# nelaturuharsha/TurboPrune

Hardware: NVIDIA H100
Metric: images_per_sec_resnet50_erk80_train_step (higher is better)
Workload: dtype bf16

## Files before the change

### include/turboprune_b200.h

```cpp
#ifndef TURBOPRUNE_B200_H
#define TURBOPRUNE_B200_H

#include <stddef.h>
#include <stdint.h>

#ifdef __cplusplus
extern "C" {
#endif

#define TP_OK                 0
#define TP_ERR_INVALID       -1
#define TP_ERR_WORKSPACE     -2
#define TP_ERR_CUDA          -3
#define TP_ERR_K_RANGE       -4
#define TP_ERR_UNSUPPORTED   -5
#define TP_ERR_DEVICE        -6

const char* tp_strerror(int code);
const char* tp_last_cuda_error(void);
int         tp_abi_version(void);
int         tp_device_sm_count(void);
int         tp_set_pdl(int on);

#define TP_SCORE_MAG      0
// ... 51 lines not shown
int tp_synth_normal(void* out, int64_t numel, uint64_t seed, uint64_t counter_offset, int raw_words, void* stream);
int tp_synth_labels(void* out, int64_t numel, int num_classes, uint64_t seed, uint64_t counter_offset, void* stream);

typedef struct tp_conv_desc {
  int32_t n, h, w, cin;
  int32_t cout, r, s;
  int32_t stride_h, stride_w, pad_h, pad_w;
  int32_t p, q;
} tp_conv_desc;

size_t tp_conv_workspace_bytes(const tp_conv_desc* d, int op);

int tp_conv_fprop(const tp_conv_desc* d, const void* x, const void* wf, const void* bias_f32,
                  void* y, void* ws, size_t ws_bytes, void* stream);
size_t tp_conv_stats_rows(const tp_conv_desc* d);
int tp_conv_fprop_stats(const tp_conv_desc* d, const void* x, const void* wf, const void* kmask_f, const void* bias_f32,
                        void* y, void* stats, void* ws, size_t ws_bytes, void* stream);
int tp_conv_dgrad(const tp_conv_desc* d, const void* dy, const void* wd, const void* kmask_d, const void* addend,
                  void* dx, void* ws, size_t ws_bytes, void* stream);
size_t tp_conv_dgrad_partial_rows(const tp_conv_desc* d);
int tp_conv_dgrad_bnrelu(const tp_conv_desc* d, const void* dy, const void* wd, const void* kmask_d,
                         const void* bn_y, const void* bn_weight, const void* bn_bias, const void* bn_mean, const void* bn_invstd,
                         void* g, void* partial, void* stream);
int tp_conv_wgrad(const tp_conv_desc* d, const void* x, const void* dy, const void* mask, const void* kmask_f,
                  int cin_real, void* dw, void* db, void* ws, size_t ws_bytes, void* stream);

int tp_bn_forward_ext(const void* y, const void* residual, void* z, int64_t M, int C,
                      const void* weight, const void* bias, void* running_mean, void* running_var,
                      void* num_batches_tracked, float momentum, float eps, int training, int relu,
                      void* save_mean, void* save_invstd, const void* ext_stats, int64_t ext_rows,
                      void* ws, size_t ws_bytes, void* stream);

size_t tp_bn_workspace_bytes(int64_t m, int c);
int tp_bn_forward(const void* y, const void* residual, void* z, int64_t m, int c,
                  const void* weight, const void* bias, void* running_mean, void* running_var,
                  void* num_batches_tracked, float momentum, float eps, int training, int relu,
                  void* save_mean, void* save_invstd, void* ws, size_t ws_bytes, void* stream);
int tp_bn_backward(const void* dz, const void* z, const void* y, int64_t m, int c, const void* weight, const void* bias,
                   const void* save_mean, const void* save_invstd, int relu, void* dy, void* dres,
                   void* dweight, void* dbias, void* ws, size_t ws_bytes, void* stream);

int tp_bn_backward_ext(const void* g, const void* y, int64_t M, int C, const void* weight, const void* bias,
                       const void* save_mean, const void* save_invstd, const void* partial_rows, int64_t n_rows,
                       void* dy, void* dweight, void* dbias, void* ws, size_t ws_bytes, void* stream);
int tp_maxpool_forward(const void* x, void* y, void* idx, int n, int h, int w, int c, int k, int stride, int pad,
                       int p, int q, void* stream);
// ... 21 lines not shown
```

### turboprune_b200/_cabi.py

```python
import ctypes
import os
from ctypes import POINTER, c_char_p, c_float, c_int, c_int32, c_int64, c_size_t, c_uint64, c_void_p

from . import build as _build

TP_SCORE_MAG, TP_SCORE_SNIP, TP_SCORE_SYNFLOW = 0, 1, 2
TP_ERR_K_RANGE = -4

_lib = None


class ConvDesc(ctypes.Structure):
    _fields_ = [(n, c_int32) for n in
                ("n", "h", "w", "cin", "cout", "r", "s", "stride_h", "stride_w", "pad_h", "pad_w", "p", "q")]


class StageItem(ctypes.Structure):
    _fields_ = [("w", c_void_p), ("mask", c_void_p), ("wf", c_void_p), ("wd", c_void_p)] + \
               [(n, c_int32) for n in ("cout", "cin", "r", "s", "cin_p", "cout_p", "wf_ld")] + \
               [("kmask_f", c_void_p), ("kmask_d", c_void_p)]


SIGNATURES = {
    "tp_strerror": (c_char_p, [c_int]),
# ... 12 lines not shown
    "tp_apply_threshold": (c_int, [POINTER(c_void_p), POINTER(c_void_p), POINTER(c_void_p), POINTER(c_void_p),
                                   POINTER(c_int64), c_int, c_int, c_void_p, c_void_p, c_size_t, c_void_p]),
    "tp_count_zeros": (c_int, [POINTER(c_void_p), POINTER(c_int64), c_int, c_void_p, c_void_p, c_size_t, c_void_p]),
    "tp_stage_weights": (c_int, [c_void_p, c_void_p, c_int, c_int, c_int, c_int, c_void_p, c_int, c_int, c_void_p, c_int,
                                 c_int, c_void_p, c_void_p, c_void_p]),
    "tp_kblock_mask_words": (c_size_t, [c_int64]),
    "tp_stage_batched_workspace_bytes": (c_size_t, [c_int]),
    "tp_stage_weights_batched": (c_int, [POINTER(StageItem), c_int, c_int, c_void_p, c_size_t, c_void_p, c_size_t, c_void_p]),
    "tp_to_nhwc_bf16": (c_int, [c_void_p, c_int, c_int64, c_int64, c_int64, c_int64, c_int, c_int, c_int, c_int,
                                c_void_p, c_int, c_void_p]),
    "tp_im2col_c8": (c_int, [c_void_p] + [c_int] * 11 + [c_void_p, c_int, c_void_p]),
    "tp_im2col_stem": (c_int, [c_void_p, c_int, c_int64, c_int64, c_int64, c_int64] + [c_int] * 13 + [c_void_p, c_int, c_void_p]),
    "tp_cifar_augment": (c_int, [c_void_p, c_void_p, c_void_p, c_void_p, c_void_p, c_void_p, c_int, c_int, c_int, c_int, c_int, c_int, c_void_p]),
    "tp_synth_normal": (c_int, [c_void_p, c_int64, c_uint64, c_uint64, c_int, c_void_p]),
    "tp_synth_labels": (c_int, [c_void_p, c_int64, c_int, c_uint64, c_uint64, c_void_p]),
    "tp_conv_workspace_bytes": (c_size_t, [POINTER(ConvDesc), c_int]),
    "tp_conv_fprop": (c_int, [POINTER(ConvDesc), c_void_p, c_void_p, c_void_p, c_void_p, c_void_p, c_size_t, c_void_p]),
    "tp_conv_stats_rows": (c_size_t, [POINTER(ConvDesc)]),
    "tp_conv_fprop_stats": (c_int, [POINTER(ConvDesc), c_void_p, c_void_p, c_void_p, c_void_p, c_void_p, c_void_p, c_void_p, c_size_t, c_void_p]),
    "tp_conv_dgrad": (c_int, [POINTER(ConvDesc), c_void_p, c_void_p, c_void_p, c_void_p, c_void_p, c_void_p, c_size_t, c_void_p]),
    "tp_conv_dgrad_partial_rows": (c_size_t, [POINTER(ConvDesc)]),
    "tp_conv_dgrad_bnrelu": (c_int, [POINTER(ConvDesc), c_void_p, c_void_p, c_void_p, c_void_p, c_void_p, c_void_p, c_void_p, c_void_p,
                                     c_void_p, c_void_p, c_void_p]),
    "tp_bn_backward_ext": (c_int, [c_void_p, c_void_p, c_int64, c_int, c_void_p, c_void_p, c_void_p, c_void_p, c_void_p, c_int64,
                                   c_void_p, c_void_p, c_void_p, c_void_p, c_size_t, c_void_p]),
    "tp_conv_wgrad": (c_int, [POINTER(ConvDesc), c_void_p, c_void_p, c_void_p, c_void_p, c_int, c_void_p, c_void_p, c_void_p,
                              c_size_t, c_void_p]),
    "tp_sgd_momentum": (c_int, [POINTER(c_void_p), POINTER(c_void_p), POINTER(c_void_p), POINTER(c_int64), c_int,
                                c_void_p, c_float, c_float, c_int, c_int, c_void_p, c_size_t, c_void_p]),
    "tp_segtable_workspace_bytes": (c_size_t, [c_int]),
    "tp_p2p_allreduce_mask": (c_int, [POINTER(c_void_p), POINTER(c_void_p), c_int, c_int, c_int64, c_void_p, c_float,
                                      c_void_p, c_int, c_int, c_void_p, c_void_p]),
    "tp_bn_workspace_bytes": (c_size_t, [c_int64, c_int]),
    "tp_bn_forward": (c_int, [c_void_p, c_void_p, c_void_p, c_int64, c_int, c_void_p, c_void_p, c_void_p, c_void_p, c_void_p,
                              c_float, c_float, c_int, c_int, c_void_p, c_void_p, c_void_p, c_size_t, c_void_p]),
    "tp_bn_forward_ext": (c_int, [c_void_p, c_void_p, c_void_p, c_int64, c_int, c_void_p, c_void_p, c_void_p, c_void_p, c_void_p,
                                  c_float, c_float, c_int, c_int, c_void_p, c_void_p, c_void_p, c_int64, c_void_p, c_size_t, c_void_p]),
    "tp_bn_backward": (c_int, [c_void_p, c_void_p, c_void_p, c_int64, c_int, c_void_p, c_void_p, c_void_p, c_void_p, c_int, c_void_p,
                               c_void_p, c_void_p, c_void_p, c_void_p, c_size_t, c_void_p]),
    "tp_maxpool_forward": (c_int, [c_void_p, c_void_p, c_void_p] + [c_int] * 9 + [c_void_p]),
    "tp_maxpool_backward": (c_int, [c_void_p, c_void_p, c_void_p] + [c_int] * 9 + [c_void_p]),
    "tp_p2p_allreduce_nvls": (c_int, [POINTER(c_void_p), POINTER(c_void_p), c_void_p, c_int, c_int, c_int64, c_void_p, c_float,
                                      c_void_p, c_int, c_void_p, c_void_p]),
}


# ... 59 lines not shown
```

### turboprune_b200/csrc/tp_core.cu

```cuda
#include "tp_common.cuh"
#include <stdlib.h>
#include <string.h>
#include <vector>

namespace tp {

static thread_local char g_last_err[512] = "";

void set_last_cuda_error(cudaError_t e, const char* where) {
  snprintf(g_last_err, sizeof(g_last_err), "%s: %s (%s)", where, cudaGetErrorName(e), cudaGetErrorString(e));
}

static int g_pdl = -1;
bool pdl_enabled() {
  if (g_pdl < 0) { const char* e = getenv("TP_PDL"); g_pdl = (e && e[0] == '1') ? 1 : 0; }
  return g_pdl == 1;
}

int sm_count() {
  static int cached[64] = {0};
  int dev = 0;
  if (cudaGetDevice(&dev) != cudaSuccess || dev < 0 || dev >= 64) return 132;
  if (cached[dev] == 0) {
    int n = 0;
// ... 52 lines not shown
  if (tiles_out) *tiles_out = tile;
  if (total_out) *total_out = start;
  return TP_OK;
}

}

extern "C" {

const char* tp_strerror(int code) {
  switch (code) {
    case TP_OK: return "ok";
    case TP_ERR_INVALID: return "invalid argument";
    case TP_ERR_WORKSPACE: return "workspace too small";
    case TP_ERR_CUDA: return "CUDA error (see tp_last_cuda_error)";
    case TP_ERR_K_RANGE: return "kthvalue(): selected number k out of range";
    case TP_ERR_UNSUPPORTED: return "unsupported configuration";
    case TP_ERR_DEVICE: return "device is not sm_90 (H100)";
    default: return "unknown error";
  }
}

const char* tp_last_cuda_error(void) { return tp::g_last_err; }
int tp_abi_version(void) { return 8; }
int tp_device_sm_count(void) { return tp::sm_count(); }
int tp_set_pdl(int on) { const int prev = tp::pdl_enabled() ? 1 : 0; tp::g_pdl = on ? 1 : 0; return prev; }

size_t tp_segtable_workspace_bytes(int n_seg) {
  return tp::align_up(sizeof(tp::Seg) * (size_t)(n_seg > 0 ? n_seg : 1), 256) + 256;
}

}
```

### turboprune_b200/csrc/tp_igemm.cu

```cuda
#include "tp_common.cuh"
#include "tp_ptx.cuh"
#include <cuda.h>
#include <mutex>

namespace tp {
using namespace ptx;

constexpr int kBlockM = 128;
constexpr int kBlockK = 64;
constexpr int kConsumers = 256;
constexpr int kThreads = kConsumers + 32;
constexpr int kProducerWarp = kConsumers / 32;
constexpr int kMaxTaps = 64;

__host__ __device__ constexpr int fwd_stages(int block_n) { return block_n == 128 ? 4 : 6; }
__host__ __device__ constexpr int fwd_tail(int block_n) { return kBlockM * block_n * 4 + 8 * 32 * 128 + 1024 + 512; }

struct TapEntry { uint16_t off_w, off_h; int32_t kofs; };

constexpr int kMaxCls = 4;

struct ClsEntry {
  int M;
  int P_it, Q_it;
// ... 3 lines not shown
  int tile0, m_groups;
};

struct FwdParams {
  int M, N;
  int ncls;
  ClsEntry cls[kMaxCls];
  int cchunks;
  int a_mode;
  int step_w, step_h;
  long long out_img_pix;
  int out_row_pix;
  int osh, osw;
  int linear;
  int ws_stages, ws_b_bytes;
  int ldc;
  int tma_store;
  __nv_bfloat16* out;
  const float* bias;
  const __nv_bfloat16* addend;
  float* stats;
  const __nv_bfloat16* bn_y;
  const float* bn_weight; const float* bn_bias; const float* bn_mean; const float* bn_invstd;
  const uint32_t* kmask;
  int kmask_words;
  TapEntry taps[kMaxTaps];
};

__device__ __forceinline__ const uint32_t* live_kmask(const uint32_t* km, int words, int N) {
#ifdef TP_NO_KMASK
  return nullptr;
#else
  if (km && __ldg(km + (size_t)((N + 63) >> 6) * words) == 0u) return nullptr;
  return km;
#endif
}

struct KSkip {
  const uint32_t* base; int words, g0, g1; int cur_w; uint32_t bits;
  __device__ __forceinline__ void begin(const uint32_t* km, int wds, int n0, int block_n, int N) {
    base = km; words = wds; cur_w = -1; bits = 0u;
    g0 = n0 >> 6; g1 = min((min(n0 + block_n, N) + 63) >> 6, ((N + 63) >> 6));
  }
  __device__ __forceinline__ bool on(int kb) {
    const int wi = kb >> 5;
    if (wi != cur_w) {
// ... 33 lines not shown
}

struct AMaps { CUtensorMap m[kMaxCls]; };

__device__ __forceinline__ void decode_tile(const FwdParams& p, int tile, int n_tiles, int& c, int& m_g, int& n_t) {
  c = 0;
#pragma unroll
  for (int j = 1; j < kMaxCls; ++j) if (j < p.ncls && tile >= p.cls[j].tile0) c = j;
  const int local = tile - p.cls[c].tile0;
  m_g = local / n_tiles; n_t = local - m_g * n_tiles;
}

template <int BLOCK_N>
__device__ __forceinline__ void fwd_mma_block(float (&acc)[BLOCK_N / 2], uint32_t a_addr, uint32_t b_addr, uint32_t accumulate) {
  const uint64_t adesc = make_smem_desc(a_addr, 16, 1024);
  const uint64_t bdesc = make_smem_desc(b_addr, 16, 1024);
#pragma unroll
  for (int k = 0; k < kBlockK / 16; ++k) {
    if constexpr (BLOCK_N == 128) wgmma_m64n128<0, 0>(acc, adesc + (uint64_t)(2 * k), bdesc + (uint64_t)(2 * k), accumulate | (uint32_t)k);
    else wgmma_m64n64<0, 0>(acc, adesc + (uint64_t)(2 * k), bdesc + (uint64_t)(2 * k), accumulate | (uint32_t)k);
  }
}

template <int BLOCK_N, bool MULTI, bool WS, bool BNB>
__global__ void __launch_bounds__(kThreads, 1)
k_igemm_fwd(const __grid_constant__ AMaps tmA, const __grid_constant__ CUtensorMap tmB,
            const __grid_constant__ FwdParams p) {
  static_assert(BLOCK_N == 64 || BLOCK_N == 128, "wgmma N of the fwd kernel");
  static_assert(!WS || !MULTI, "weight-stationary walk: single class");
  static_assert(!BNB || (!MULTI && !WS), "BatchNorm-backward epilogue: single class, default walk");
  constexpr int kABytes = kBlockM * kBlockK * 2;
  constexpr int kBBytes = BLOCK_N * kBlockK * 2;
  constexpr int kStageBytes = kABytes + kBBytes;
  constexpr int kStages = fwd_stages(BLOCK_N);
  extern __shared__ __align__(1024) uint8_t smem_raw[];
  uint8_t* smem = (uint8_t*)(((uintptr_t)smem_raw + 1023) & ~(uintptr_t)1023);
  pdl_trigger();
  constexpr int kStgBytes = 32 * 128;
  constexpr int kMaxStages = 16;
  const int n_stages = WS ? p.ws_stages : kStages;
  const int a_stride = WS ? kABytes : kStageBytes;
  uint8_t* const a_base = WS ? smem + p.ws_b_bytes : smem;
  float* const acc_tile = (float*)(a_base + n_stages * a_stride);
  uint8_t* stg_base = (uint8_t*)(acc_tile + kBlockM * BLOCK_N);
  uint64_t* full_bar = (uint64_t*)(stg_base + 8 * kStgBytes);
  uint64_t* empty_bar = full_bar + (WS ? kMaxStages : kStages);
  uint64_t* bres_bar = empty_bar + (WS ? kMaxStages : kStages);

  const int warp = threadIdx.x >> 5, lane = threadIdx.x & 31;
  const int n_tiles = (p.N + BLOCK_N - 1) / BLOCK_N;
  const int total_tiles = p.cls[p.ncls - 1].tile0 + p.cls[p.ncls - 1].m_groups * n_tiles;
  const int ws_nt = WS ? (int)blockIdx.x % n_tiles : 0;
  const int ws_m0 = WS ? (int)blockIdx.x / n_tiles : 0, ws_dm = WS ? (int)gridDim.x / n_tiles : 1;
// ... 182 lines not shown
            const int r = r0 + 8 * h, col = 8 * j + 2 * (lane & 3);
            *reinterpret_cast<float2*>(acc_tile + r * BLOCK_N + (((col >> 2) ^ (r & 7)) << 2) + (col & 3)) =
                make_float2(acc[4 * j + 2 * h], acc[4 * j + 2 * h + 1]);
          }
        bar_sync(1, kConsumers);
      }
      if (p.tma_store) {
        const uint32_t buf = smem_u32(stg_base + warp * kStgBytes);
        __nv_bfloat16* const gout = p.out;
        const __nv_bfloat16* const gadd = p.addend;
        {
        const float* bias = p.bias;
        float* stats = p.stats ? p.stats + (long long)(m_t * 4 + quarter) * 2 * N + c16 * 8 : nullptr;
        const uint32_t wr_base = buf + lane * 128;
        const uint32_t wr_sw = (uint32_t)(lane & 7);
        const uint32_t rd_even = buf + r_in * 128 + ((uint32_t)(c16 ^ r_in) << 4);
        const uint32_t rd_odd = buf + (r_in + 4) * 128 + ((uint32_t)(c16 ^ (r_in + 4)) << 4);
        uint4 a_pref[8];
#pragma unroll 1
        for (int c = half * 64; c < BLOCK_N; c += 128) {
          const int n0 = n_t * BLOCK_N + c;
          if (n0 >= N) break;
          const bool col_ok = n0 + c16 * 8 + 8 <= N;
          uint32_t v[64];
          acc_row_ld(c, v);
          acc_row_ld(c + 32, v + 32);
          if (gadd) {
            if (c == half * 64) {
#pragma unroll
              for (int i = 0; i < 8; ++i) {
                a_pref[i] = make_uint4(0u, 0u, 0u, 0u);
                if (i * 4 + r_in < rows_left && col_ok) a_pref[i] = *reinterpret_cast<const uint4*>(gadd + row_off(i) + n0);
              }
            }
#pragma unroll
            for (int i = 0; i < 8; ++i) sts128(((i & 1) ? rd_odd : rd_even) + (uint32_t)((i >> 1) * 1024), a_pref[i]);
            if (c + 128 < BLOCK_N && n0 + 128 < N) {
              const bool col_ok2 = n0 + 128 + c16 * 8 + 8 <= N;
#pragma unroll
              for (int i = 0; i < 8; ++i) {
                a_pref[i] = make_uint4(0u, 0u, 0u, 0u);
                if (i * 4 + r_in < rows_left && col_ok2) a_pref[i] = *reinterpret_cast<const uint4*>(gadd + row_off(i) + n0 + 128);
              }
            }
            __syncwarp();
          }
// ... 64 lines not shown
                  const float2 y2 = __bfloat1622float2(yh[q]);
                  if (!(fmaf(y2.x, sc[2 * q], sf[2 * q]) > 0.f)) d2.x = 0.f;
                  if (!(fmaf(y2.y, sc[2 * q + 1], sf[2 * q + 1]) > 0.f)) d2.y = 0.f;
                  gh[q] = __floats2bfloat162_rn(d2.x, d2.y);
                  s1[2 * q] += d2.x;     s2[2 * q] = fmaf(d2.x, (y2.x - nm[2 * q]) * is_[2 * q], s2[2 * q]);
                  s1[2 * q + 1] += d2.y; s2[2 * q + 1] = fmaf(d2.y, (y2.y - nm[2 * q + 1]) * is_[2 * q + 1], s2[2 * q + 1]);
                }
              }
            }
#pragma unroll
            for (int i = 0; i < 8; ++i)
              if (i * 4 + r_in < rows_left && col_ok) *reinterpret_cast<uint4*>(gout + row_off(i) + n0) = o[i];
#pragma unroll
            for (int q = 0; q < 8; ++q) {
              s1[q] += __shfl_xor_sync(0xffffffffu, s1[q], 8);  s2[q] += __shfl_xor_sync(0xffffffffu, s2[q], 8);
              s1[q] += __shfl_xor_sync(0xffffffffu, s1[q], 16); s2[q] += __shfl_xor_sync(0xffffffffu, s2[q], 16);
            }
            if (r_in == 0 && col_ok) {
              float4* d1 = reinterpret_cast<float4*>(stats + n0);
              float4* d2 = reinterpret_cast<float4*>(stats + N + n0);
              d1[0] = make_float4(s1[0], s1[1], s1[2], s1[3]); d1[1] = make_float4(s1[4], s1[5], s1[6], s1[7]);
              d2[0] = make_float4(s2[0], s2[1], s2[2], s2[3]); d2[1] = make_float4(s2[4], s2[5], s2[6], s2[7]);
            }
          } else {
#pragma unroll
          for (int i = 0; i < 8; ++i)
            if (i * 4 + r_in < rows_left && col_ok) *reinterpret_cast<uint4*>(gout + row_off(i) + n0) = o[i];
          if (stats) {
            float s1[8], s2[8];
#pragma unroll
            for (int q = 0; q < 8; ++q) { s1[q] = 0.f; s2[q] = 0.f; }
#pragma unroll
            for (int i = 0; i < 8; ++i) {
              if (i * 4 + r_in < rows_left) {
                const __nv_bfloat162* h2 = reinterpret_cast<const __nv_bfloat162*>(&o[i]);
#pragma unroll
                for (int q = 0; q < 4; ++q) {
                  const float2 t2 = __bfloat1622float2(h2[q]);
                  s1[2 * q] += t2.x; s2[2 * q] = fmaf(t2.x, t2.x, s2[2 * q]);
                  s1[2 * q + 1] += t2.y; s2[2 * q + 1] = fmaf(t2.y, t2.y, s2[2 * q + 1]);
                }
              }
            }
#pragma unroll
            for (int q = 0; q < 8; ++q) {
              s1[q] += __shfl_xor_sync(0xffffffffu, s1[q], 8);  s2[q] += __shfl_xor_sync(0xffffffffu, s2[q], 8);
// ... 377 lines not shown
static int pick_block_n(long long m_tiles, int n) {
  const int sms = sm_count();
  if (const char* e = getenv("TP_IGEMM_BN")) {
    const int f = atoi(e);
    if ((f == 64 || f == 128) && (f == 64 || n > f / 2)) return f;
  }
  int best = 64; double best_score = -1;
  const int cands[2] = {128, 64};
  const double weight[2] = {1.0, 0.82};
  for (int i = 0; i < 2; ++i) {
    int bn = cands[i];
    if (bn > 64 && n <= bn / 2) continue;
    long long tiles = m_tiles * ((n + bn - 1) / bn);
    long long waves = (tiles + sms - 1) / sms;
    double eff = (double)tiles / (double)(waves * sms) * weight[i];
    if (eff > best_score) { best_score = eff; best = bn; }
  }
  return best;
}

constexpr int kSmemMax = 232448;
constexpr int kWsMinStages = 3;

template <int BN, bool MULTI, bool WS, bool BNB = false>
static int launch_fwd(const AMaps& a, const CUtensorMap& b, FwdParams& p, cudaStream_t st) {
  constexpr int kStages = fwd_stages(BN);
  constexpr int kTail = fwd_tail(BN);
  int smem = kStages * (kBlockM * kBlockK * 2 + BN * kBlockK * 2) + kTail;
  static_assert(fwd_stages(BN) * (kBlockM * kBlockK * 2 + BN * kBlockK * 2) + fwd_tail(BN) <= kSmemMax, "fwd smem budget");
  const int n_tiles = (p.N + BN - 1) / BN;
  if (WS) {
    p.ws_b_bytes = p.cls[0].ntaps * p.cchunks * BN * kBlockK * 2;
    p.ws_stages = (kSmemMax - kTail - p.ws_b_bytes) / (kBlockM * kBlockK * 2);
    if (p.ws_stages > 16) p.ws_stages = 16;
    if (p.ws_stages < kWsMinStages) return TP_ERR_UNSUPPORTED;
    smem = p.ws_b_bytes + p.ws_stages * kBlockM * kBlockK * 2 + kTail;
  }
  static bool attr_set = false;
  if (!attr_set) {
    TP_CUDA_CHECK(cudaFuncSetAttribute(k_igemm_fwd<BN, MULTI, WS, BNB>, cudaFuncAttributeMaxDynamicSharedMemorySize, WS ? kSmemMax : smem));
    attr_set = true;
  }
  long long ctiles = 0;
  for (int c = 0; c < p.ncls; ++c) {
    p.cls[c].m_groups = (int)((p.cls[c].M + kBlockM - 1) / kBlockM);
    if (ctiles > 0x7fffffffll) return TP_ERR_UNSUPPORTED;
    p.cls[c].tile0 = (int)ctiles;
    ctiles += (long long)p.cls[c].m_groups * n_tiles;
  }
  if (ctiles > 0x7fffffffll || ctiles <= 0) return TP_ERR_UNSUPPORTED;
  int grid = (int)(ctiles < sm_count() ? ctiles : sm_count());
  if (WS) grid = (sm_count() / n_tiles) * n_tiles;
  TP_CUDA_CHECK(launch(k_igemm_fwd<BN, MULTI, WS, BNB>, dim3(grid), dim3(kThreads), (size_t)smem, st, a, b, p));
  TP_LAUNCH_CHECK();
  return TP_OK;
}

static int run_fwd(const AMaps& a, const CUtensorMap& b, FwdParams& p, int bn, cudaStream_t st) {
  p.linear = p.ncls == 1 && p.osh == 1 && p.osw == 1 && p.cls[0].oah == 0 && p.cls[0].oaw == 0 &&
             p.out_row_pix == p.cls[0].Q_it && p.out_img_pix == (long long)p.cls[0].P_it * p.cls[0].Q_it;
  p.tma_store = (p.ldc % 8 == 0 && p.N % 8 == 0 && (((uintptr_t)p.out) & 15) == 0 &&
                 (!p.addend || (((uintptr_t)p.addend) & 15) == 0)) ? 1 : 0;
  if (p.stats && !(p.tma_store && p.linear)) return TP_ERR_UNSUPPORTED;
  const bool multi = !p.linear;
  if (multi) {
    if (bn == 128) return launch_fwd<128, true, false>(a, b, p, st);
    return launch_fwd<64, true, false>(a, b, p, st);
  }
  if (p.bn_y) {
    if (!p.tma_store || !p.stats) return TP_ERR_UNSUPPORTED;
    if (bn == 128) return launch_fwd<128, false, false, true>(a, b, p, st);
    return launch_fwd<64, false, false, true>(a, b, p, st);
  }
  const int n_tiles = (p.N + bn - 1) / bn;
  const long long m_tiles = (p.cls[0].M + kBlockM - 1) / kBlockM;
  const long long b_bytes = (long long)p.cls[0].ntaps * p.cchunks * bn * kBlockK * 2;
  const long long ws_max_b = (long long)kSmemMax - (bn == 128 ? fwd_tail(128) : fwd_tail(64)) - kWsMinStages * kBlockM * kBlockK * 2;
  const char* e = getenv("TP_IGEMM_WS");
  const bool ws = e && atoi(e) != 0 && b_bytes <= ws_max_b && n_tiles <= sm_count() / 2 && m_tiles >= 4ll * (sm_count() / n_tiles);
  if (ws) {
    if (bn == 128) return launch_fwd<128, false, true>(a, b, p, st);
    return launch_fwd<64, false, true>(a, b, p, st);
  }
  if (bn == 128) return launch_fwd<128, false, false>(a, b, p, st);
  return launch_fwd<64, false, false>(a, b, p, st);
}

template <int NB>
static int launch_wgrad(int grid, const CUtensorMap& ta, const CUtensorMap& tb, const WgParams& p, cudaStream_t st) {
  constexpr int smem = 4 * (kBlockM * kBlockK * 2 + 4 * 64 * kBlockK * 2) + 1024 + 256;
// ... 67 lines not shown
    TapEntry& t = p.taps[r * d->s + s];
    t.off_w = (uint16_t)s; t.off_h = (uint16_t)r; t.kofs = (r * d->s + s) * d->cin;
  }
  AMaps ta; CUtensorMap tb;
  if (is_plain_gemm(d)) {
    p.a_mode = 0;
    rc = make_tiled_map(&ta.m[0], x, (uint64_t)d->cin, (uint64_t)p.M, (uint64_t)d->cin, kBlockM); if (rc) return rc;
  } else {
    p.a_mode = 1;
    ce.base_w = -d->pad_w; ce.base_h = -d->pad_h; p.step_w = d->stride_w; p.step_h = d->stride_h;
    rc = make_im2col_map(&ta.m[0], x, d->n, d->h, d->w, d->cin, ce.base_w, ce.base_h, p.step_w, p.step_h, d->p, d->q, kBlockM);
    if (rc) return rc;
  }
  for (int c = 1; c < kMaxCls; ++c) ta.m[c] = ta.m[0];
  const int bn = pick_block_n((p.M + kBlockM - 1) / kBlockM, p.N);
  rc = make_tiled_map(&tb, wf, (uint64_t)d->r * d->s * d->cin, (uint64_t)d->cout, (uint64_t)d->r * d->s * d->cin, (uint32_t)bn);
  if (rc) return rc;
  return run_fwd(ta, tb, p, bn, st);
}

struct BnGate { const void* y; const float* weight; const float* bias; const float* mean; const float* invstd; float* partial; };

static int conv_dgrad_impl(const tp_conv_desc* d, const void* dy, const void* wd, const void* kmask_d, const void* addend,
                           void* dx, const BnGate* gate, void* stream);

int tp_conv_dgrad(const tp_conv_desc* d, const void* dy, const void* wd, const void* kmask_d, const void* addend,
                  void* dx, void* ws, size_t ws_bytes, void* stream) {
  (void)ws; (void)ws_bytes;
  return conv_dgrad_impl(d, dy, wd, kmask_d, addend, dx, nullptr, stream);
}

int tp_conv_dgrad_bnrelu(const tp_conv_desc* d, const void* dy, const void* wd, const void* kmask_d,
                         const void* bn_y, const void* bn_weight, const void* bn_bias, const void* bn_mean, const void* bn_invstd,
                         void* g, void* partial, void* stream) {
  if (!d || !bn_y || !bn_mean || !bn_invstd || !partial) return TP_ERR_INVALID;
  if (d->stride_h != 1 || d->stride_w != 1 || d->cin % 8 != 0) return TP_ERR_UNSUPPORTED;
  if ((((uintptr_t)bn_y) | ((uintptr_t)bn_weight) | ((uintptr_t)bn_bias) | ((uintptr_t)bn_mean) | ((uintptr_t)bn_invstd) | ((uintptr_t)partial)) & 15)
    return TP_ERR_UNSUPPORTED;
  BnGate bn = {bn_y, (const float*)bn_weight, (const float*)bn_bias, (const float*)bn_mean, (const float*)bn_invstd, (float*)partial};
  return conv_dgrad_impl(d, dy, wd, kmask_d, nullptr, g, &bn, stream);
}

size_t tp_conv_dgrad_partial_rows(const tp_conv_desc* d) {
  if (!d) return 0;
  const long long M = (long long)d->n * d->h * d->w;
  return (size_t)((M + kBlockM - 1) / kBlockM) * 4;
}

static int conv_dgrad_impl(const tp_conv_desc* d, const void* dy, const void* wd, const void* kmask_d, const void* addend,
                           void* dx, const BnGate* gate, void* stream) {
  if (!d || !dy || !wd || !dx) return TP_ERR_INVALID;
  const int cop = d->cout;
  if (cop % 8 != 0 || d->r * d->s > kMaxTaps) return TP_ERR_UNSUPPORTED;
  if (d->r * d->s > 1 && cop % 64 != 0) return TP_ERR_UNSUPPORTED;
  int rc = load_driver_fns(); if (rc) return rc;
  rc = bind_device_of(d ? (const void*)dy : nullptr); if (rc) return rc;
  cudaStream_t st = (cudaStream_t)stream;
  const int R = d->r, S = d->s;
  const long long ktot = (long long)R * S * cop;
  const int sh = d->stride_h, sw = d->stride_w;
  FwdParams p = {};
  p.N = d->cin;
  p.cchunks = (cop + 63) / 64;
  p.out_img_pix = (long long)d->h * d->w; p.out_row_pix = d->w;
  p.ldc = d->cin; p.out = (__nv_bfloat16*)dx; p.bias = nullptr; p.addend = (const __nv_bfloat16*)addend;
  p.kmask = (const uint32_t*)kmask_d; p.kmask_words = (int)tp_kblock_mask_words(ktot);
  p.step_w = 1; p.step_h = 1;
  if (gate) {
    p.bn_y = (const __nv_bfloat16*)gate->y; p.bn_weight = gate->weight; p.bn_bias = gate->bias; p.bn_mean = gate->mean; p.bn_invstd = gate->invstd;
    p.stats = gate->partial;
  }
  AMaps ta; CUtensorMap tb;
  if (sh == 1 && sw == 1) {
    p.M = d->n * d->h * d->w;
    p.ncls = 1; p.osh = 1; p.osw = 1;
    ClsEntry& ce = p.cls[0];
    ce.M = p.M; ce.P_it = d->h; ce.Q_it = d->w; ce.ntaps = R * S; ce.tap0 = 0; ce.oah = 0; ce.oaw = 0;
    for (int r = 0; r < R; ++r) for (int s = 0; s < S; ++s) {
      TapEntry& t = p.taps[r * S + s];
      t.off_w = (uint16_t)s; t.off_h = (uint16_t)r; t.kofs = (r * S + s) * cop;
    }
    if (is_plain_gemm(d)) {
      p.a_mode = 0;
      rc = make_tiled_map(&ta.m[0], dy, (uint64_t)cop, (uint64_t)p.M, (uint64_t)cop, kBlockM); if (rc) return rc;
    } else {
      p.a_mode = 1;
      ce.base_w = -(S - 1 - d->pad_w); ce.base_h = -(R - 1 - d->pad_h);
      rc = make_im2col_map(&ta.m[0], dy, d->n, d->p, d->q, cop, ce.base_w, ce.base_h, 1, 1, d->h, d->w, kBlockM);
      if (rc) return rc;
    }
    for (int c = 1; c < kMaxCls; ++c) ta.m[c] = ta.m[0];
  } else {
    if (sh * sw > kMaxCls || R * S > kMaxTaps) return TP_ERR_UNSUPPORTED;
    p.a_mode = 1; p.osh = sh; p.osw = sw;
// ... 116 lines not shown
```

### turboprune_b200/fused_norm.py

```python
import types
from ctypes import c_void_p

import torch
import torch.nn as nn

from . import _cabi, ops
from .utils.mask_layers import grad_slots


def _ptr(t):
    return c_void_p(t.data_ptr()) if t is not None else None


_PARTIALS = {}


def offer_partials(g, partial, token):
    _PARTIALS[g.data_ptr()] = (partial, token, g, g._version)


def drop_partials():
    _PARTIALS.clear()


# ... 19 lines not shown
            rc = lib.tp_bn_forward_ext(_ptr(xn), _ptr(rn), _ptr(z), m, c, _ptr(weight), _ptr(bias), _ptr(running_mean),
                                       _ptr(running_var), _ptr(nbt), float(momentum), float(eps), int(training), int(relu),
                                       _ptr(save_mean), _ptr(save_invstd), _ptr(ext_stats) if use_ext else None,
                                       ext_stats.shape[0] if use_ext else 0, _ptr(wsb), wsb.numel(), _cabi.stream_ptr(dev))
        _cabi.check(rc, "tp_bn_forward")
        ops._count(3 if training else 2)
        if training:
            ctx.relu = 0 if not relu else (1 if residual is not None else 2)
            ctx.save_for_backward(xn, z.permute(0, 2, 3, 1) if ctx.relu == 1 else None, weight, bias, save_mean, save_invstd)
            ctx.has_res = residual is not None
            ctx.res_dtype = residual.dtype if residual is not None else None
            ctx.x_dtype = x.dtype
        return z

    @staticmethod
    def backward(ctx, dz):
        lib = _cabi.load()
        xn, z, weight, bias, save_mean, save_invstd = ctx.saved_tensors
        n, h, w, c = xn.shape
        m = n * h * w
        dev = xn.device
        dzn = ops.to_nhwc_bf16(dz, c)
        dy = torch.empty_like(xn)
        dres = torch.empty_like(xn) if ctx.has_res else None
        ws_, bs_ = ctx.grad_slots if ctx.grad_slots is not None else (None, None)
        direct = ws_ is not None and bs_ is not None
        dweight = ws_ if direct else torch.empty(c, dtype=torch.float32, device=dev)
        dbias = bs_ if direct else torch.empty(c, dtype=torch.float32, device=dev)
        wsb = ops._workspace(lib.tp_bn_workspace_bytes(m, c), dev, "bn")
        hint = _PARTIALS.pop(dzn.data_ptr(), None) if _PARTIALS else None
        if hint is not None and (hint[1] is not ctx.token or hint[2]._version != hint[3] or ctx.relu != 2 or ctx.has_res):
            hint = None
        with torch.cuda.device(dev):
            if hint is not None:
                rc = lib.tp_bn_backward_ext(_ptr(dzn), _ptr(xn), m, c, _ptr(weight), _ptr(bias), _ptr(save_mean), _ptr(save_invstd),
                                            _ptr(hint[0]), hint[0].shape[0], _ptr(dy), _ptr(dweight), _ptr(dbias), _ptr(wsb),
                                            wsb.numel(), _cabi.stream_ptr(dev))
            else:
                rc = lib.tp_bn_backward(_ptr(dzn), _ptr(z), _ptr(xn), m, c, _ptr(weight), _ptr(bias), _ptr(save_mean), _ptr(save_invstd),
                                        int(ctx.relu), _ptr(dy), _ptr(dres), _ptr(dweight), _ptr(dbias), _ptr(wsb), wsb.numel(),
                                        _cabi.stream_ptr(dev))
        _cabi.check(rc, "tp_bn_backward")
        ops._count(3)
        gx = dy.permute(0, 3, 1, 2)
        if gx.dtype != ctx.x_dtype:
            gx = gx.to(ctx.x_dtype)
        gr = dres.permute(0, 3, 1, 2) if dres is not None else None
        if gr is not None and gr.dtype != ctx.res_dtype:
            gr = gr.to(ctx.res_dtype)
        if direct:
            dweight = dbias = None
            ops.grad_ready(ws_, bs_)
        return gx, gr, dweight, dbias, None, None, None, None, None, None, None, None, None, None


class BatchNorm2dB200(nn.BatchNorm2d):

    def forward(self, x, residual=None, relu=False, ext_stats=None):
        training = self.training or not self.track_running_stats
        if (not x.is_cuda or x.shape[1] % 8 != 0 or (not training and torch.is_grad_enabled() and x.requires_grad)
                or (self.momentum is None and training and self.track_running_stats)):
            y = super().forward(x)
            if residual is not None:
                y = y + residual
            return torch.relu(y) if relu else y
        momentum = 0.0 if self.momentum is None else self.momentum
        slots = grad_slots(self.weight, self.bias)
        saved = None
        if training and relu and residual is None and ops.BN_BWD_FUSION and torch.is_grad_enabled():
            c = x.shape[1]
            with torch.no_grad():
                xn = ops.to_nhwc_bf16(x.detach(), c)
            saved = (xn, torch.empty(c, dtype=torch.float32, device=x.device),
                     torch.empty(c, dtype=torch.float32, device=x.device), object())
        z = _BNFn.apply(x, residual, self.weight, self.bias, self.running_mean, self.running_var,
                        self.num_batches_tracked if (training and self.track_running_stats) else None,
                        momentum, self.eps, training, relu, slots, ext_stats, saved)
        if saved is not None:
            z._tp_bn_src = (saved[0], self.weight, self.bias, saved[1], saved[2], saved[3])
        return z


class _MaxPoolFn(torch.autograd.Function):
    @staticmethod
    def forward(ctx, x, k, stride, pad):
        lib = _cabi.load()
        n, c, h, w = x.shape
        xn = ops.to_nhwc_bf16(x, c)
        p = (h + 2 * pad - k) // stride + 1
        q = (w + 2 * pad - k) // stride + 1
        y = ops.empty_cl(n, c, p, q, x.device)
        idx = torch.empty(n, p, q, c, dtype=torch.uint8, device=x.device)
        with torch.cuda.device(x.device):
            rc = lib.tp_maxpool_forward(_ptr(xn), _ptr(y), _ptr(idx), n, h, w, c, k, stride, pad, p, q, _cabi.stream_ptr(x.device))
        _cabi.check(rc, "tp_maxpool_forward")
        ops._count()
        ctx.save_for_backward(idx)
        ctx.geom = (n, h, w, c, k, stride, pad, p, q)
        ctx.x_dtype = x.dtype
        return y

    @staticmethod
# ... 128 lines not shown
```

### turboprune_b200/ops.py

```python
import ctypes
from ctypes import c_void_p

import torch

from . import _cabi

_launches = 0


def _count(n=1):
    global _launches
    _launches += n


def launch_count() -> int:
    return _launches


class KernelTimer:

    def __init__(self):
        self.records = []

    def totals(self):
# ... 488 lines not shown

def set_bn_bwd_fusion(on: bool):
    global BN_BWD_FUSION
    BN_BWD_FUSION = bool(on)


def conv_dgrad_bnrelu(desc, dy_nhwc, wd, bn_src, kmask=None):
    lib = _cabi.load()
    dev = dy_nhwc.device
    y, weight, bias, mean, invstd = bn_src[:5]
    g = torch.empty(desc.n, desc.h, desc.w, desc.cin, dtype=torch.bfloat16, device=dev)
    rows = int(lib.tp_conv_dgrad_partial_rows(ctypes.byref(desc)))
    partial = torch.empty(rows, 2, desc.cin, dtype=torch.float32, device=dev)
    km = (kmask if kmask is not None else getattr(wd, "kmask", None)) if KBLOCK_SKIP else None
    P = lambda t: c_void_p(t.data_ptr()) if t is not None else None
    with torch.cuda.device(dev), _Timed("dgrad", desc):
        rc = lib.tp_conv_dgrad_bnrelu(ctypes.byref(desc), P(dy_nhwc), P(wd), P(km), P(y), P(weight), P(bias), P(mean), P(invstd),
                                      P(g), P(partial), _cabi.stream_ptr(dev))
    if rc == -5:
        return None
    _cabi.check(rc, "tp_conv_dgrad_bnrelu")
    _count()
    return g, partial


def conv_wgrad(desc, x_nhwc, dy_nhwc, mask4d, cin_real, want_db=False, dw_out=None, db_out=None, kmask=None):
    lib = _cabi.load()
    dev = x_nhwc.device
    dw = dw_out if dw_out is not None else torch.empty(desc.cout, cin_real, desc.r, desc.s, dtype=torch.float32, device=dev)
    db = (db_out if db_out is not None else torch.empty(desc.cout, dtype=torch.float32, device=dev)) if want_db else None
    nbytes = lib.tp_conv_workspace_bytes(ctypes.byref(desc), 2)
    wsb = _workspace(nbytes, dev, "wgrad")
    with torch.cuda.device(dev), _Timed("wgrad", desc):
        km = kmask if KBLOCK_SKIP else None
        rc = lib.tp_conv_wgrad(ctypes.byref(desc), c_void_p(x_nhwc.data_ptr()), c_void_p(dy_nhwc.data_ptr()),
                               c_void_p(mask4d.data_ptr()), c_void_p(km.data_ptr()) if km is not None else None,
                               cin_real, c_void_p(dw.data_ptr()),
                               c_void_p(db.data_ptr()) if db is not None else None,
                               c_void_p(wsb.data_ptr()), wsb.numel(), _cabi.stream_ptr(dev))
    _cabi.check(rc, "tp_conv_wgrad")
    _count(3 if want_db else 2)
    return dw, db


class MaskedConv2dFn(torch.autograd.Function):

# ... 26 lines not shown
                wf, wd = stage_weights(w32, m32, cg, False, wf_ld=kp)
            y = empty_cl(n, cout, desc.p, desc.q, x.device)
            if want_stats:
                _, stats = conv_fprop(gdesc, xg, wf, bias, out=y, want_stats=True)
            else:
                conv_fprop(gdesc, xg, wf, bias, out=y)
            ctx.mode = "stem"
            ctx.gdesc = gdesc
            ctx.save_for_backward(xg, m32)
        else:
            xn = to_nhwc_bf16(x, cin_p)
            if (staged is not None and staged[0].shape == (cout, r * s * cin_p)
                    and (not need_dx or (staged[1] is not None and staged[1].shape == (cin, r * s * cout_p)))):
                wf, wd = staged
            else:
                wf, wd = stage_weights(w32, m32, cin_p, need_dx, cout_p)
            y = empty_cl(n, cout, desc.p, desc.q, x.device)
            if want_stats:
                _, stats = conv_fprop(desc, xn, wf, bias, out=y, want_stats=True)
            else:
                conv_fprop(desc, xn, wf, bias, out=y)
            ctx.mode = "conv"
            ctx.save_for_backward(xn, m32, wd)
            if (bn_src is not None and BN_BWD_FUSION and need_dx and not want_skip and stride == (1, 1) and cin_p == cin
                    and bn_src[0].shape == xn.shape):
                ctx.bn_src = bn_src
            ctx.wd_kmask = getattr(wd, "kmask", None) if wd is not None else None
            ctx.wf_kmask = getattr(wf, "kmask", None)
        ctx.desc = desc
        ctx.cin = cin
        ctx.has_bias = bias is not None
        ctx.cout_p = cout_p
        ctx.x_dtype = x.dtype
        if want_skip:
            if want_stats:
                ctx.mark_non_differentiable(stats)
                return y, x, stats
            return y, x
        if want_stats:
            ctx.mark_non_differentiable(stats)
            return y, stats
        return y

    @staticmethod
    def backward(ctx, dy, *rest):
        dskip = rest[0] if ctx.want_skip and rest else None
        desc = ctx.desc
        if dy is None:
# ... 9 lines not shown
            if need_dw:
                r, s = desc.r, desc.s
                cin = m32.shape[1]
                ones = torch.ones(cout, xg.shape[1], dtype=torch.float32, device=xg.device)
                gd = ctx.gdesc
                dwm, db = conv_wgrad(gd, xg, dyn.view(-1, cout), ones.view(cout, -1, 1, 1), xg.shape[1], need_db)
                cg = stem_geometry(cin, r, s)[0]
                dw = dwm[:, :r * s * cg].reshape(cout, r * s, cg)[:, :, :cin].permute(0, 2, 1).reshape(cout, cin, r, s) * m32
        else:
            xn, m32, wd = ctx.saved_tensors
            cin = ctx.cin
            ddesc = desc
            if ctx.cout_p != cout:
                ddesc = _cabi.ConvDesc(desc.n, desc.h, desc.w, desc.cin, ctx.cout_p, desc.r, desc.s, desc.stride_h,
                                       desc.stride_w, desc.pad_h, desc.pad_w, desc.p, desc.q)
            if need_dx:
                addend = None
                if dskip is not None:
                    addend = to_nhwc_bf16(dskip, cin)
                xdesc = ddesc if cin == desc.cin else _cabi.ConvDesc(desc.n, desc.h, desc.w, cin, ctx.cout_p, desc.r, desc.s,
                                                                      desc.stride_h, desc.stride_w, desc.pad_h, desc.pad_w,
                                                                      desc.p, desc.q)
                fused = None
                if ctx.bn_src is not None and addend is None:
                    fused = conv_dgrad_bnrelu(xdesc, dyn, wd, ctx.bn_src, kmask=ctx.wd_kmask)
                if fused is not None:
                    g, partial = fused
                    from . import fused_norm
                    fused_norm.offer_partials(g, partial, ctx.bn_src[5])
                    dx = g.permute(0, 3, 1, 2)
                else:
                    dx = conv_dgrad(xdesc, dyn, wd, addend, kmask=ctx.wd_kmask).permute(0, 3, 1, 2)
                if dx.dtype != ctx.x_dtype:
                    dx = dx.to(ctx.x_dtype)
            if need_dw:
                if ctx.cout_p != cout:
                    m_p = torch.zeros(ctx.cout_p, *m32.shape[1:], dtype=torch.float32, device=m32.device)
                    m_p[:cout] = m32
                    dwp, dbp = conv_wgrad(ddesc, xn, dyn, m_p, cin, need_db)
                    dw = dwp[:cout].contiguous()
                    db = dbp[:cout].contiguous() if dbp is not None else None
                else:
                    ws_, bs_ = ctx.grad_slots if ctx.grad_slots is not None else (None, None)
                    direct_w = ws_ is not None and ws_.is_contiguous() and ws_.numel() == m32.numel()
                    direct_b = need_db and bs_ is not None
                    if WGRAD_SIDE_STREAM and direct_w and (direct_b or not need_db):
                        dev = xn.device
# ... 39 lines not shown
```

Baseline: 6341.

## Fuse ReLU gating of residual-block output into the consuming conv's dgrad epilogue

Adds a dgrad epilogue variant (BNR) that reads the post-ReLU activation z and zeroes gradient elements where z <= 0, so the ReLU backward after a residual add happens inside the conv dgrad kernel. BatchNorm backward then skips its relu/dres pass and reuses the gated gradient directly as the residual gradient. This is meant to remove a separate elementwise pass and a dres buffer write per residual block. The cost is an extra z load in the epilogue, a new kernel instantiation, and more complex partial-handoff logic in Python.

Result: faster. 6504 (median of 6 runs) (+2.6%).

```diff
diff --git a/include/turboprune_b200.h b/include/turboprune_b200.h
--- a/include/turboprune_b200.h
+++ b/include/turboprune_b200.h
@@ -97,6 +97,8 @@
 int tp_conv_dgrad_bnrelu(const tp_conv_desc* d, const void* dy, const void* wd, const void* kmask_d,
                          const void* bn_y, const void* bn_weight, const void* bn_bias, const void* bn_mean, const void* bn_invstd,
                          void* g, void* partial, void* stream);
+int tp_conv_dgrad_gate(const tp_conv_desc* d, const void* dy, const void* wd, const void* kmask_d, const void* addend,
+                       const void* z, void* g, void* stream);
 int tp_conv_wgrad(const tp_conv_desc* d, const void* x, const void* dy, const void* mask, const void* kmask_f,
                   int cin_real, void* dw, void* db, void* ws, size_t ws_bytes, void* stream);
 
diff --git a/turboprune_b200/_cabi.py b/turboprune_b200/_cabi.py
--- a/turboprune_b200/_cabi.py
+++ b/turboprune_b200/_cabi.py
@@ -58,6 +58,7 @@
     "tp_conv_dgrad_partial_rows": (c_size_t, [POINTER(ConvDesc)]),
     "tp_conv_dgrad_bnrelu": (c_int, [POINTER(ConvDesc), c_void_p, c_void_p, c_void_p, c_void_p, c_void_p, c_void_p, c_void_p, c_void_p,
                                      c_void_p, c_void_p, c_void_p]),
+    "tp_conv_dgrad_gate": (c_int, [POINTER(ConvDesc)] + [c_void_p] * 7),
     "tp_bn_backward_ext": (c_int, [c_void_p, c_void_p, c_int64, c_int, c_void_p, c_void_p, c_void_p, c_void_p, c_void_p, c_int64,
                                    c_void_p, c_void_p, c_void_p, c_void_p, c_size_t, c_void_p]),
     "tp_conv_wgrad": (c_int, [POINTER(ConvDesc), c_void_p, c_void_p, c_void_p, c_void_p, c_int, c_void_p, c_void_p, c_void_p,
diff --git a/turboprune_b200/csrc/tp_core.cu b/turboprune_b200/csrc/tp_core.cu
--- a/turboprune_b200/csrc/tp_core.cu
+++ b/turboprune_b200/csrc/tp_core.cu
@@ -98,7 +98,7 @@
 }
 
 const char* tp_last_cuda_error(void) { return tp::g_last_err; }
-int tp_abi_version(void) { return 8; }
+int tp_abi_version(void) { return 9; }
 int tp_device_sm_count(void) { return tp::sm_count(); }
 int tp_set_pdl(int on) { const int prev = tp::pdl_enabled() ? 1 : 0; tp::g_pdl = on ? 1 : 0; return prev; }
 
diff --git a/turboprune_b200/csrc/tp_igemm.cu b/turboprune_b200/csrc/tp_igemm.cu
--- a/turboprune_b200/csrc/tp_igemm.cu
+++ b/turboprune_b200/csrc/tp_igemm.cu
@@ -49,6 +49,7 @@
   float* stats;
   const __nv_bfloat16* bn_y;
   const float* bn_weight; const float* bn_bias; const float* bn_mean; const float* bn_invstd;
+  const __nv_bfloat16* bn_z;
   const uint32_t* kmask;
   int kmask_words;
   TapEntry taps[kMaxTaps];
@@ -128,13 +129,14 @@
   }
 }
 
-template <int BLOCK_N, bool MULTI, bool WS, bool BNB>
+template <int BLOCK_N, bool MULTI, bool WS, bool BNB, bool BNR>
 __global__ void __launch_bounds__(kThreads, 1)
 k_igemm_fwd(const __grid_constant__ AMaps tmA, const __grid_constant__ CUtensorMap tmB,
             const __grid_constant__ FwdParams p) {
   static_assert(BLOCK_N == 64 || BLOCK_N == 128, "wgmma N of the fwd kernel");
   static_assert(!WS || !MULTI, "weight-stationary walk: single class");
-  static_assert(!BNB || (!MULTI && !WS), "BatchNorm-backward epilogue: single class, default walk");
+  static_assert(!(BNB || BNR) || (!MULTI && !WS), "BatchNorm-backward epilogue: single class, default walk");
+  static_assert(!(BNB && BNR), "one gate source");
   constexpr int kABytes = kBlockM * kBlockK * 2;
   constexpr int kBBytes = BLOCK_N * kBlockK * 2;
   constexpr int kStageBytes = kABytes + kBBytes;
@@ -363,6 +365,14 @@
           const int n0 = n_t * BLOCK_N + c;
           if (n0 >= N) break;
           const bool col_ok = n0 + c16 * 8 + 8 <= N;
+          uint4 zv[8];
+          if (BNR) {
+#pragma unroll
+            for (int i = 0; i < 8; ++i) {
+              zv[i] = make_uint4(0u, 0u, 0u, 0u);
+              if (i * 4 + r_in < rows_left && col_ok) zv[i] = *reinterpret_cast<const uint4*>(p.bn_z + row_off(i) + n0);
+            }
+          }
           uint32_t v[64];
           acc_row_ld(c, v);
           acc_row_ld(c + 32, v + 32);
@@ -473,6 +483,23 @@
               d1[0] = make_float4(s1[0], s1[1], s1[2], s1[3]); d1[1] = make_float4(s1[4], s1[5], s1[6], s1[7]);
               d2[0] = make_float4(s2[0], s2[1], s2[2], s2[3]); d2[1] = make_float4(s2[4], s2[5], s2[6], s2[7]);
             }
+          } else if (BNR) {
+#pragma unroll
+            for (int i = 0; i < 8; ++i) {
+              __nv_bfloat162* gh = reinterpret_cast<__nv_bfloat162*>(&o[i]);
+              const __nv_bfloat162* zh = reinterpret_cast<const __nv_bfloat162*>(&zv[i]);
+#pragma unroll
+              for (int q = 0; q < 4; ++q) {
+                float2 d2 = __bfloat1622float2(gh[q]);
+                const float2 z2 = __bfloat1622float2(zh[q]);
+                if (!(z2.x > 0.f)) d2.x = 0.f;
+                if (!(z2.y > 0.f)) d2.y = 0.f;
+                gh[q] = __floats2bfloat162_rn(d2.x, d2.y);
+              }
+            }
+#pragma unroll
+            for (int i = 0; i < 8; ++i)
+              if (i * 4 + r_in < rows_left && col_ok) *reinterpret_cast<uint4*>(gout + row_off(i) + n0) = o[i];
           } else {
 #pragma unroll
           for (int i = 0; i < 8; ++i)
@@ -896,7 +923,7 @@
 constexpr int kSmemMax = 232448;
 constexpr int kWsMinStages = 3;
 
-template <int BN, bool MULTI, bool WS, bool BNB = false>
+template <int BN, bool MULTI, bool WS, bool BNB = false, bool BNR = false>
 static int launch_fwd(const AMaps& a, const CUtensorMap& b, FwdParams& p, cudaStream_t st) {
   constexpr int kStages = fwd_stages(BN);
   constexpr int kTail = fwd_tail(BN);
@@ -912,7 +939,7 @@
   }
   static bool attr_set = false;
   if (!attr_set) {
-    TP_CUDA_CHECK(cudaFuncSetAttribute(k_igemm_fwd<BN, MULTI, WS, BNB>, cudaFuncAttributeMaxDynamicSharedMemorySize, WS ? kSmemMax : smem));
+    TP_CUDA_CHECK(cudaFuncSetAttribute(k_igemm_fwd<BN, MULTI, WS, BNB, BNR>, cudaFuncAttributeMaxDynamicSharedMemorySize, WS ? kSmemMax : smem));
     attr_set = true;
   }
   long long ctiles = 0;
@@ -925,7 +952,7 @@
   if (ctiles > 0x7fffffffll || ctiles <= 0) return TP_ERR_UNSUPPORTED;
   int grid = (int)(ctiles < sm_count() ? ctiles : sm_count());
   if (WS) grid = (sm_count() / n_tiles) * n_tiles;
-  TP_CUDA_CHECK(launch(k_igemm_fwd<BN, MULTI, WS, BNB>, dim3(grid), dim3(kThreads), (size_t)smem, st, a, b, p));
+  TP_CUDA_CHECK(launch(k_igemm_fwd<BN, MULTI, WS, BNB, BNR>, dim3(grid), dim3(kThreads), (size_t)smem, st, a, b, p));
   TP_LAUNCH_CHECK();
   return TP_OK;
 }
@@ -940,6 +967,11 @@
   if (multi) {
     if (bn == 128) return launch_fwd<128, true, false>(a, b, p, st);
     return launch_fwd<64, true, false>(a, b, p, st);
+  }
+  if (p.bn_z) {
+    if (!p.tma_store) return TP_ERR_UNSUPPORTED;
+    if (bn == 128) return launch_fwd<128, false, false, false, true>(a, b, p, st);
+    return launch_fwd<64, false, false, false, true>(a, b, p, st);
   }
   if (p.bn_y) {
     if (!p.tma_store || !p.stats) return TP_ERR_UNSUPPORTED;
@@ -1053,12 +1085,12 @@
 struct BnGate { const void* y; const float* weight; const float* bias; const float* mean; const float* invstd; float* partial; };
 
 static int conv_dgrad_impl(const tp_conv_desc* d, const void* dy, const void* wd, const void* kmask_d, const void* addend,
-                           void* dx, const BnGate* gate, void* stream);
+                           void* dx, const BnGate* gate, const void* gate_z, void* stream);
 
 int tp_conv_dgrad(const tp_conv_desc* d, const void* dy, const void* wd, const void* kmask_d, const void* addend,
                   void* dx, void* ws, size_t ws_bytes, void* stream) {
   (void)ws; (void)ws_bytes;
-  return conv_dgrad_impl(d, dy, wd, kmask_d, addend, dx, nullptr, stream);
+  return conv_dgrad_impl(d, dy, wd, kmask_d, addend, dx, nullptr, nullptr, stream);
 }
 
 int tp_conv_dgrad_bnrelu(const tp_conv_desc* d, const void* dy, const void* wd, const void* kmask_d,
@@ -1069,7 +1101,14 @@
   if ((((uintptr_t)bn_y) | ((uintptr_t)bn_weight) | ((uintptr_t)bn_bias) | ((uintptr_t)bn_mean) | ((uintptr_t)bn_invstd) | ((uintptr_t)partial)) & 15)
     return TP_ERR_UNSUPPORTED;
   BnGate bn = {bn_y, (const float*)bn_weight, (const float*)bn_bias, (const float*)bn_mean, (const float*)bn_invstd, (float*)partial};
-  return conv_dgrad_impl(d, dy, wd, kmask_d, nullptr, g, &bn, stream);
+  return conv_dgrad_impl(d, dy, wd, kmask_d, nullptr, g, &bn, nullptr, stream);
+}
+
+int tp_conv_dgrad_gate(const tp_conv_desc* d, const void* dy, const void* wd, const void* kmask_d, const void* addend,
+                       const void* z, void* g, void* stream) {
+  if (!d || !z) return TP_ERR_INVALID;
+  if (d->stride_h != 1 || d->stride_w != 1 || d->cin % 8 != 0 || (((uintptr_t)z) & 15)) return TP_ERR_UNSUPPORTED;
+  return conv_dgrad_impl(d, dy, wd, kmask_d, addend, g, nullptr, z, stream);
 }
 
 size_t tp_conv_dgrad_partial_rows(const tp_conv_desc* d) {
@@ -1079,7 +1118,7 @@
 }
 
 static int conv_dgrad_impl(const tp_conv_desc* d, const void* dy, const void* wd, const void* kmask_d, const void* addend,
-                           void* dx, const BnGate* gate, void* stream) {
+                           void* dx, const BnGate* gate, const void* gate_z, void* stream) {
   if (!d || !dy || !wd || !dx) return TP_ERR_INVALID;
   const int cop = d->cout;
   if (cop % 8 != 0 || d->r * d->s > kMaxTaps) return TP_ERR_UNSUPPORTED;
@@ -1101,6 +1140,7 @@
     p.bn_y = (const __nv_bfloat16*)gate->y; p.bn_weight = gate->weight; p.bn_bias = gate->bias; p.bn_mean = gate->mean; p.bn_invstd = gate->invstd;
     p.stats = gate->partial;
   }
+  p.bn_z = (const __nv_bfloat16*)gate_z;
   AMaps ta; CUtensorMap tb;
   if (sh == 1 && sw == 1) {
     p.M = d->n * d->h * d->w;
diff --git a/turboprune_b200/fused_norm.py b/turboprune_b200/fused_norm.py
--- a/turboprune_b200/fused_norm.py
+++ b/turboprune_b200/fused_norm.py
@@ -65,24 +65,25 @@
         dev = xn.device
         dzn = ops.to_nhwc_bf16(dz, c)
         dy = torch.empty_like(xn)
-        dres = torch.empty_like(xn) if ctx.has_res else None
         ws_, bs_ = ctx.grad_slots if ctx.grad_slots is not None else (None, None)
         direct = ws_ is not None and bs_ is not None
         dweight = ws_ if direct else torch.empty(c, dtype=torch.float32, device=dev)
         dbias = bs_ if direct else torch.empty(c, dtype=torch.float32, device=dev)
         wsb = ops._workspace(lib.tp_bn_workspace_bytes(m, c), dev, "bn")
         hint = _PARTIALS.pop(dzn.data_ptr(), None) if _PARTIALS else None
-        if hint is not None and (hint[1] is not ctx.token or hint[2]._version != hint[3] or ctx.relu != 2 or ctx.has_res):
+        if hint is not None and (hint[1] is not ctx.token or hint[2]._version != hint[3]):
             hint = None
+        gated = hint is not None and hint[0] is None
+        dres = (dzn if gated else torch.empty_like(xn)) if ctx.has_res else None
         with torch.cuda.device(dev):
-            if hint is not None:
+            if hint is not None and not gated:
                 rc = lib.tp_bn_backward_ext(_ptr(dzn), _ptr(xn), m, c, _ptr(weight), _ptr(bias), _ptr(save_mean), _ptr(save_invstd),
                                             _ptr(hint[0]), hint[0].shape[0], _ptr(dy), _ptr(dweight), _ptr(dbias), _ptr(wsb),
                                             wsb.numel(), _cabi.stream_ptr(dev))
             else:
                 rc = lib.tp_bn_backward(_ptr(dzn), _ptr(z), _ptr(xn), m, c, _ptr(weight), _ptr(bias), _ptr(save_mean), _ptr(save_invstd),
-                                        int(ctx.relu), _ptr(dy), _ptr(dres), _ptr(dweight), _ptr(dbias), _ptr(wsb), wsb.numel(),
-                                        _cabi.stream_ptr(dev))
+                                        0 if gated else int(ctx.relu), _ptr(dy), None if gated else _ptr(dres), _ptr(dweight),
+                                        _ptr(dbias), _ptr(wsb), wsb.numel(), _cabi.stream_ptr(dev))
         _cabi.check(rc, "tp_bn_backward")
         ops._count(3)
         gx = dy.permute(0, 3, 1, 2)
@@ -110,7 +111,7 @@
         momentum = 0.0 if self.momentum is None else self.momentum
         slots = grad_slots(self.weight, self.bias)
         saved = None
-        if training and relu and residual is None and ops.BN_BWD_FUSION and torch.is_grad_enabled():
+        if training and relu and ops.BN_BWD_FUSION and torch.is_grad_enabled():
             c = x.shape[1]
             with torch.no_grad():
                 xn = ops.to_nhwc_bf16(x.detach(), c)
@@ -120,7 +121,7 @@
                         self.num_batches_tracked if (training and self.track_running_stats) else None,
                         momentum, self.eps, training, relu, slots, ext_stats, saved)
         if saved is not None:
-            z._tp_bn_src = (saved[0], self.weight, self.bias, saved[1], saved[2], saved[3])
+            z._tp_bn_src = (saved[0], self.weight, self.bias, saved[1], saved[2], saved[3], residual is not None)
         return z
 
 
diff --git a/turboprune_b200/ops.py b/turboprune_b200/ops.py
--- a/turboprune_b200/ops.py
+++ b/turboprune_b200/ops.py
@@ -534,6 +534,21 @@
     _cabi.check(rc, "tp_conv_dgrad_bnrelu")
     _count()
     return g, partial
+
+
+def conv_dgrad_gate(desc, dy_nhwc, wd, addend, z_nhwc, kmask=None):
+    lib = _cabi.load()
+    dev = dy_nhwc.device
+    g = torch.empty(desc.n, desc.h, desc.w, desc.cin, dtype=torch.bfloat16, device=dev)
+    km = (kmask if kmask is not None else getattr(wd, "kmask", None)) if KBLOCK_SKIP else None
+    P = lambda t: c_void_p(t.data_ptr()) if t is not None else None
+    with torch.cuda.device(dev), _Timed("dgrad", desc):
+        rc = lib.tp_conv_dgrad_gate(ctypes.byref(desc), P(dy_nhwc), P(wd), P(km), P(addend), P(z_nhwc), P(g), _cabi.stream_ptr(dev))
+    if rc == -5:
+        return None
+    _cabi.check(rc, "tp_conv_dgrad_gate")
+    _count()
+    return g
 
 
 def conv_wgrad(desc, x_nhwc, dy_nhwc, mask4d, cin_real, want_db=False, dw_out=None, db_out=None, kmask=None):
@@ -606,8 +621,8 @@
                 conv_fprop(desc, xn, wf, bias, out=y)
             ctx.mode = "conv"
             ctx.save_for_backward(xn, m32, wd)
-            if (bn_src is not None and BN_BWD_FUSION and need_dx and not want_skip and stride == (1, 1) and cin_p == cin
-                    and bn_src[0].shape == xn.shape):
+            if (bn_src is not None and BN_BWD_FUSION and need_dx and (bn_src[6] or not want_skip) and stride == (1, 1)
+                    and cin_p == cin and bn_src[0].shape == xn.shape):
                 ctx.bn_src = bn_src
             ctx.wd_kmask = getattr(wd, "kmask", None) if wd is not None else None
             ctx.wf_kmask = getattr(wf, "kmask", None)
@@ -663,7 +678,10 @@
                                                                       desc.stride_h, desc.stride_w, desc.pad_h, desc.pad_w,
                                                                       desc.p, desc.q)
                 fused = None
-                if ctx.bn_src is not None and addend is None:
+                if ctx.bn_src is not None and ctx.bn_src[6]:
+                    g = conv_dgrad_gate(xdesc, dyn, wd, addend, xn, kmask=ctx.wd_kmask)
+                    fused = (g, None) if g is not None else None
+                elif ctx.bn_src is not None and addend is None:
                     fused = conv_dgrad_bnrelu(xdesc, dyn, wd, ctx.bn_src, kmask=ctx.wd_kmask)
                 if fused is not None:
                     g, partial = fused
```
